# prsinha1/Distributed-Inverse-Problem-Admm

Hardware: AMD Instinct MI355X
Metric: ADMM node-updates/sec (whole node), 512² phantom; rel-Fro vs CPU ref (higher is better)
Workload: dtype f32 samples / f64 state; 1 GPU; C3 (BASELINE.json configs[2] 512^2, 16 graph nodes (ring), 96 angles/node, float32 samples, iso TV, lam=0.02 rho=2, split-Bregman 10x5 CG) on 1 GPU(s), one step = one outer ADMM iteration; image=512, nodes=16, angles_per_node=96, graph=ring, parallelism=graph-node shards x1, batch_streams=1

## Files before the change

distributed-inverse-problem-admm_amd/csrc/admm_tomo.hip:

```cpp
#include <hip/hip_runtime.h>

#include <algorithm>
#include <cmath>
#include <cstdio>
#include <cstdlib>
#include <cstring>
#include <initializer_list>
#include <memory>
#include <string>
#include <type_traits>
#include <utility>
#include <vector>

#include "../../include/admm_tomo.h"
#include "fwd_plan.hpp"
#include "kernels.hpp"

using namespace admm;

static_assert(sizeof(FgBlock) == sizeof(int4) && alignof(FgBlock) == alignof(int4), "FgBlock must be an int4");

namespace {
thread_local std::string g_err;

// ... 145 lines not shown
  int kbias = 0;
  int wexp = 0;
  static constexpr int kPlans = kFwdPlans;
  FwdPlan plans[kPlans];
  Buf plan_groups_b[kPlans], plan_rng_b[kPlans];
  const FgGroup* plan_groups(int pl) const { return plan_groups_b[pl].as<const FgGroup>(); }
  const FgRange* plan_rng(int pl) const { return plan_rng_b[pl].as<const FgRange>(); }
  int plan_n[kPlans] = {}, plan_blocks[kPlans] = {};
  double plan_staged[kPlans] = {};
  const FgGroup* groups = nullptr;
  const FgRange* rng = nullptr;
  int n_groups = 0;
  bool mirror_half = false;
  Buf fg_order;
  int fg_nblk = 0, fg_order_nch = 0;
  int fg_cpb = 1;
  Stream cap;

  bool csr = false;
  long long nnz = 0;
  Buf f_ptr, f_idx, f_val, t_ptr, t_idx, t_val;

  Buf op_img, op_imgT, op_sino, op_fpart;
  Buf op_order[kPlans];
  int op_nblk[kPlans] = {};
  int op_fpart_key = -1;

  bool bound = false;
  admm_batch b{};
  int vb = 1;
  bool mm = false;
  int bk_staging = 0;
  bool bk_epi_lds = true;
  int n_cu = 0;
  std::unique_ptr<admm_ctx> half;
  Buf xs, xsT, p, pT, Hp, sino, bI, fpart, r, c, d2, e2;
  Buf dsumS;
  Buf wS;
  bool weighted = false;
  Buf x2, p2;
  Buf pring;
  Buf ats;
  std::vector<Event>* tf_ev = nullptr;
  size_t tf_next = 0;
  int tf_kind = 0;
  bool ats_valid = false;
  Buf partH, partS, partD, partE;
  Buf redH;
  int P_back = 0, P_tile = 0, P_fwd = 0, P_edge = 0;
  Graph upd, upd_reuse, cons;

  admm_ctx() = default;
  admm_ctx(const admm_ctx&) = delete;
  admm_ctx& operator=(const admm_ctx&) = delete;
  ~admm_ctx() {
    scope.enter(device);
    (void)hipDeviceSynchronize();
    half.reset();
  }
};

namespace {

int vb_for(int V, int dtype) {
  const int vb = V >= 5 ? 8 : (V >= 3 ? 4 : (V == 2 ? 2 : 1));
  return dtype == ADMM_DTYPE_F64 ? std::min(vb, 4) : vb;
// ... 230 lines not shown
    const size_t mthreads = (size_t)mh * (MODE == 0 ? 2 : 1);
    dim3 mg((unsigned)((mthreads + kBlock - 1) / kBlock), nch * (VB / MH));
    with_weights(wts, [&](auto... w) {
      hipLaunchKernelGGL((k_fwd_combine_mirror<T, VBV, VB, MODE, decltype(w)...>), mg, dim3(kBlock), 0, s,
                         (const T*)C->fpart.p, sino, b, part, C->half->fang(), C->g.n_det, C->half->g.n_angles, V, w...);
    });
    CHECK_LAUNCH();
    return ADMM_OK;
  }
  dim3 cg((C->mrays + kBlock - 1) / kBlock, nch);
  with_weights(wts, [&](auto... w) {
    hipLaunchKernelGGL((k_fwd_combine<T, VB, MODE, decltype(w)...>), cg, dim3(kBlock), 0, s, (const T*)C->fpart.p, sino, b,
                       part, C->fang(), C->g.n_det, C->g.n_angles, V, w...);
  });
  CHECK_LAUNCH();
  return ADMM_OK;
}

template <typename T>
void back_geom(BackArgs<T>& a, const admm_ctx* C, const admm_ctx* A, int V) {
  a.ang = A->bang();
  a.angc = A->bangc();
  a.K = A->Kb;
  a.kbias = A->kbias;
  a.wexp = A->wexp;
  a.N = C->g.N;
  a.n_det = C->g.n_det;
  a.n_ang = A->g.n_angles;
  a.V = V;
}

template <typename T, int VB, int MODE>
int launch_back(admm_ctx* C, BackArgs<T> a, int V, hipStream_t s) {
  if constexpr (MODE == BACK_H || MODE == BACK_INIT || MODE == BACK_DIAG || MODE == BACK_ATB) {
    if (C->mm) {
      constexpr int VBV = mirror_vb<T, VB>(), MH = VBV / 2;
      back_geom(a, C, C->half.get(), V);
      const int N = C->g.N, Nh = (N + 1) / 2;
      dim3 grid((N + kBTJ - 1) / kBTJ, (Nh + kBTI - 1) / kBTI, ((V + VB - 1) / VB) * (VB / MH));
      void (*kern)(BackArgs<T>) = k_back_mirror<T, VBV, VB, MODE>;
      if constexpr (back_mirror_dma<T, VBV, MODE>()) {
        if (C->bk_staging == 1) {
          kern = k_back_mirror_reg<T, VBV, VB, MODE>;
        } else if constexpr (std::is_same<T, float>::value) {
          const bool fills = (long)grid.x * grid.y * grid.z >= 2L * C->n_cu;
          if (grid.z % 2 == 0 && (C->bk_staging == 3 || (C->bk_staging == 0 && fills))) {
            kern = C->bk_epi_lds ? k_back_mirror_2<T, VBV, VB> : k_back_mirror_2_gepi<T, VBV, VB>;
            grid.z /= 2;
          } else if (!C->bk_epi_lds) {
            kern = k_back_mirror_gepi<T, VBV, VB, MODE>;
          }
        }
      }
      hipLaunchKernelGGL(kern, grid, dim3(kBkThreads), 0, s, a);
      CHECK_LAUNCH();
      return ADMM_OK;
    }
  }
  back_geom(a, C, C, V);
  const int N = C->g.N;
  constexpr bool kOneImage = MODE == BACK_WSQ || MODE == BACK_WSQW;
  dim3 grid((N + kBTJ - 1) / kBTJ, (N + kBTI - 1) / kBTI, kOneImage ? 1 : (V + VB - 1) / VB);
  if (C->csr) {
    a.csr_ptr = (const int*)C->t_ptr.p;
    a.csr_idx = (const int*)C->t_idx.p;
    a.csr_val = (const T*)C->t_val.p;
    hipLaunchKernelGGL((k_back<T, VB, MODE, true>), grid, dim3(kBkThreads), 0, s, a);
// ... 156 lines not shown
      std::swap(dcur, dnxt);
      std::swap(ecur, enxt);
    }
    std::swap(xcur, xnxt);
    if (!last) std::swap(slot[0], slot[F == 2 ? K : 1]);
  }
  if (xcur != B.x_ext)
    HIPCHK(hipMemcpyAsync(B.x_ext, xcur, (size_t)V * npix * sizeof(double), hipMemcpyDeviceToDevice, s));
  if (dcur != B.d) {
    HIPCHK(hipMemcpyAsync(B.d, dcur, 2 * V * npix * sizeof(double), hipMemcpyDeviceToDevice, s));
    HIPCHK(hipMemcpyAsync(B.e, ecur, 2 * V * npix * sizeof(double), hipMemcpyDeviceToDevice, s));
  }
  RET((launch_fwd_batch<T, VB, 1>(C, xs, xsT, sino, (const T*)B.b, (double*)C->partS.p, V, s)));
  {
    BackArgs<T> a{};
    a.sino = sino;
    a.part = (double*)C->partD.p;
    a.dsum = B.dsum;
    a.cvec = c;
    a.x = B.x_ext;
    a.phantom = B.phantom;
    a.edges = edge_in(B);
    a.qv = B.q;
    a.inc_off = B.inc_off;
    a.inc_edge = B.inc_edge;
    a.inc_qslot = B.inc_qslot;
    a.inc_sign = B.inc_sign;
    a.rho = B.rho;
    a.lam = B.lam;
    a.mu = B.mu;
    a.tv_kind = B.tv_kind;
    a.evar = B.e;
    a.out_t = (B.flags & ADMM_BATCH_KEEP_X) ? (T*)C->ats.p : nullptr;
    RET((launch_back<T, VB, BACK_DIAG>(C, a, V, s)));
  }
  RET(launch_reduce((double*)C->partS.p, V, C->P_fwd, B.node_stats, 1, ADMM_NODE_STATS, ADMM_NODE_STAT_MSE_SINO, s));
  RET(launch_reduce((double*)C->partD.p, 5 * V, Pb, B.node_stats, 5, ADMM_NODE_STATS, ADMM_NODE_STAT_G2, s));
  return ADMM_OK;
}

int enqueue_update_any(admm_ctx* C, hipStream_t s, bool reuse = false, int rounds = 0) {
  return with_type_vb(C->dtype, C->vb, [&](auto tt, auto vbc) {
    return enqueue_update<typename decltype(tt)::type, decltype(vbc)::value>(C, s, reuse, rounds);
  });
}

int cons_rows(int n_xext) { return n_xext <= 16 ? 16 : n_xext <= 64 ? 64 : n_xext <= 128 ? 128 : 0; }

int enqueue_consensus_stored(admm_ctx* C, int e0, int e1, hipStream_t s) {
  const admm_batch& B = C->b;
  if (e1 <= e0) return ADMM_OK;
  const int npix = C->npix;
  dim3 grid((npix + kBlock * 4 - 1) / (kBlock * 4), e1 - e0);
  hipLaunchKernelGGL(k_consensus<false>, grid, dim3(kBlock), 0, s, B.x_ext, B.y, nullptr, B.z, nullptr, B.edge_a,
                     B.edge_b, (double*)C->partE.p, npix, e0);
  CHECK_LAUNCH();
  RET(launch_reduce((double*)C->partE.p + (size_t)3 * e0 * C->P_edge, 3 * (e1 - e0), C->P_edge,
                    B.edge_stats + (size_t)3 * e0, 1, 1, 0, s));
  return ADMM_OK;
}

int enqueue_consensus(admm_ctx* C, hipStream_t s) {
  const admm_batch& B = C->b;
  if (B.n_edges == 0) return ADMM_OK;
  const int npix = C->npix;
  if (B.z == nullptr) {
    const dim3 g((npix + kConsPix - 1) / kConsPix);
// ... 106 lines not shown
  RET(ensure(C->op_sino, vbmax * m * ds));
  RET(ensure(C->op_fpart, (size_t)kFgSeg * vbmax * m * ds));
  for (int v0 = 0; v0 < nimg; v0 += step) {
    const int nc = std::min(step, nimg - v0);
    const T* in = img + (size_t)v0 * npix;
    T* out = sino + (size_t)v0 * m;
    RET(with_vb(vb_for(nc, C->dtype), [&](auto vbc) { return op_forward_chunk<T, decltype(vbc)::value>(C, in, out, nc, s); }));
  }
  return ADMM_OK;
}

}

extern "C" {

int admm_abi_version(void) { return ADMM_ABI_VERSION; }
const char* admm_last_error(void) { return g_err.c_str(); }

int admm_ctx_create(admm_ctx** out, const admm_geom* geom, int dtype, int max_images, int device) {
  if (!out || !geom) return fail(ADMM_E_INVALID, "null argument");
  *out = nullptr;
  const admm_geom g = *geom;
  if (const char* err = check_geom(g, dtype, max_images)) return fail(ADMM_E_INVALID, err);
  GeomTables T;
  if (const char* err = geom_tables(g, dtype, T)) return fail(ADMM_E_INVALID, err);
  FwdPlans P = build_fwd_plans(g, T.fa);
  DEVICE_SCOPE(device);
  std::unique_ptr<admm_ctx> C(new admm_ctx());
  C->g = g;
  C->dtype = dtype;
  C->device = device;
  C->bk_staging = env_word("ADMM_BK_STAGING", {"reg", "dma1", "dma2"});
  C->bk_epi_lds = env_word("ADMM_BK_EPI", {"global"}) == 0;
  HIPCHK(hipDeviceGetAttribute(&C->n_cu, hipDeviceAttributeMultiprocessorCount, device));
  C->max_images = max_images;
  C->npix = g.N * g.N;
  C->mrays = g.n_angles * g.n_det;
  C->Kb = T.Kb;
  C->kbias = T.kbias;
  C->wexp = T.wexp;
  RET(upload(C->fang_b, T.fa));
  RET(upload(C->bang_b, T.ba));
  RET(upload(C->bangc_b, T.bc));
  if (P.fits) {
    for (int pl = 0; pl < admm_ctx::kPlans; ++pl) {
      FwdPlan& Q = P.plan[pl];
      if (Q.groups.empty()) continue;
      RET(upload(C->plan_groups_b[pl], Q.groups));
      RET(upload(C->plan_rng_b[pl], Q.ranges));
      C->plan_n[pl] = (int)Q.groups.size();
      C->plan_blocks[pl] = (int)Q.blocks.size();
      C->plan_staged[pl] = Q.staged;
      C->plans[pl] = std::move(Q);
    }
    select_fwd_plan(C.get(), 0);
  }
  HIPCHK(hipStreamCreateWithFlags(&C->cap.s, hipStreamNonBlocking));
  *out = C.release();
  return ADMM_OK;
}

int admm_ctx_create_matrix(admm_ctx** out, int N, int m, long long nnz, const long long* indptr,
                           const int* indices, const double* values, int dtype, int max_images, int device) {
  if (!out || !indptr || (nnz > 0 && (!indices || !values))) return fail(ADMM_E_INVALID, "null argument");
  *out = nullptr;
  if (N < 2 || N > 4096 || m < 1) return fail(ADMM_E_INVALID, "bad matrix sizes");
// ... 5 lines not shown
    return fail(ADMM_E_INVALID, "batch too large for 32-bit buffer offsets; split it across contexts");
  if (indptr[0] != 0 || indptr[m] != nnz) return fail(ADMM_E_INVALID, "indptr must run from 0 to nnz");
  for (int r = 0; r < m; ++r)
    if (indptr[r + 1] < indptr[r]) return fail(ADMM_E_INVALID, "indptr not non-decreasing");
  for (long long k = 0; k < nnz; ++k)
    if (indices[k] < 0 || (size_t)indices[k] >= npix) return fail(ADMM_E_INVALID, "column index out of range");
  std::vector<int> tptr(npix + 1, 0), tidx((size_t)nnz);
  std::vector<double> tval((size_t)nnz);
  for (long long k = 0; k < nnz; ++k) ++tptr[(size_t)indices[k] + 1];
  for (size_t c = 0; c < npix; ++c) tptr[c + 1] += tptr[c];
  {
    std::vector<int> fill(tptr.begin(), tptr.end() - 1);
    for (int r = 0; r < m; ++r)
      for (long long k = indptr[r]; k < indptr[r + 1]; ++k) {
        const int q = fill[indices[k]]++;
        tidx[q] = r;
        tval[q] = values[k];
      }
  }
  std::vector<int> fptr(m + 1);
  for (int r = 0; r <= m; ++r) fptr[r] = (int)indptr[r];
  DEVICE_SCOPE(device);
  std::unique_ptr<admm_ctx> C(new admm_ctx());
  C->g = admm_geom{};
  C->g.N = N;
  C->g.n_angles = 1;
  C->g.n_det = m;
  C->dtype = dtype;
  C->device = device;
  C->max_images = max_images;
  C->npix = (int)npix;
  C->mrays = m;
  C->csr = true;
  C->nnz = nnz;
  FwdAngle fa{};
  fa.L = 1.0;
  BackAngle ba{};
  BackAngleC bc{};
  auto upv = [&](Buf& b, const std::vector<double>& v) {
    if (dtype == ADMM_DTYPE_F64) return upload(b, v, 16);
    return upload(b, std::vector<float>(v.begin(), v.end()), 16);
  };
  RET(upload(C->f_ptr, fptr, 16));
  RET(upload(C->f_idx, indices, (size_t)nnz * 4, 16));
  RET(upv(C->f_val, std::vector<double>(values, values + nnz)));
  RET(upload(C->t_ptr, tptr, 16));
  RET(upload(C->t_idx, tidx, 16));
  RET(upv(C->t_val, tval));
  RET(upload(C->fang_b, &fa, sizeof(fa)));
  RET(upload(C->bang_b, &ba, sizeof(ba)));
  RET(upload(C->bangc_b, &bc, sizeof(bc)));
  HIPCHK(hipStreamCreateWithFlags(&C->cap.s, hipStreamNonBlocking));
  *out = C.release();
  return ADMM_OK;
}

int admm_ctx_destroy(admm_ctx* C) {
  if (!C) return ADMM_OK;
  delete C;
  return ADMM_OK;
}

int admm_project_fwd(admm_ctx* C, const void* img, void* sino, int nimg, void* stream) {
  if (!C || !img || !sino) return fail(ADMM_E_INVALID, "null argument");
  if (nimg < 1 || nimg > C->max_images) return fail(ADMM_E_INVALID, "nimg out of range");
  hipStream_t s = (hipStream_t)stream;
// ... 384 lines not shown
```

distributed-inverse-problem-admm_amd/csrc/kernels.hpp:

```cpp
#pragma once
#include <hip/hip_runtime.h>
#include <stdint.h>

#include <type_traits>

#include "tables.hpp"

namespace admm {

constexpr int kBlock = 256;
constexpr int kTile = 32;
constexpr int kFwdRays = 64;
constexpr int kFwdSegs = 8;
constexpr int kFwdBlock = kFwdRays * kFwdSegs;


__device__ __forceinline__ int clampi(int v, int lo, int hi) { return min(max(v, lo), hi); }

constexpr double kKfBias = 1048576.0;
constexpr unsigned kKfHi = 0x41300000u;
__device__ __forceinline__ void kf_split(double kfb, unsigned& hi, float& fu) {
  const uint64_t b = __builtin_bit_cast(uint64_t, kfb);
  hi = (unsigned)(b >> 32);
  fu = (float)(unsigned)b;
// ... 1002 lines not shown
        } else {
          lo[u] = T(0);
          hi[u] = T(0);
        }
      } else if constexpr (WT) {
        lo[u] *= wl[u];
        hi[u] *= wh[u];
      }
    }
    T* base = sino + (size_t)rc * m_full * VBR + mq * MH;
    gstore<T, MH>(base + ray * VBR, lo);
    gstore<T, MH>(base + ray2 * VBR, hi);
  }
  if (MODE == 1) {
    __shared__ double lds[4 * MH];
    block_reduce<MH>(sq, lds);
    if (threadIdx.x == 0) {
#pragma unroll
      for (int u = 0; u < MH; ++u)
        if (vr0 + u < V) pout[(size_t)(vr0 + u) * gridDim.x + blockIdx.x] = sq[u];
    }
  }
}

struct EdgeIn {
  const double* z;
  const double* y;
  const double* yb;
  const double* xp;
  const int* ea;
  const int* eb;
};

enum BackMode { BACK_PLAIN = 0, BACK_ATB = 1, BACK_WSQ = 2, BACK_H = 3, BACK_INIT = 4, BACK_DIAG = 5, BACK_WSQW = 6 };

template <typename T>
struct BackArgs {
  const T* sino;
  const BackAngle* ang;
  const BackAngleC* angc;
  double K;
  int kbias;
  int wexp;
  int N, n_det, n_ang, V;
  const int* csr_ptr;
  const int* csr_idx;
  const T* csr_val;
  T* out_t;
  double* out_d;
  double* part;
  const T* pin;
  const double* r;
  const double* dsum;
  const T* dsum_s;
  const double* atb;
  const double* cvec;
  const double* dvar;
  const double* evar;
  const double* x;
  const double* phantom;
  EdgeIn edges;
  const double* qv;
  const int* inc_off;
  const int* inc_edge;
  const int* inc_qslot;
  const int* inc_sign;
  double rho, lam, mu;
// ... 201 lines not shown
    gstore<T, VB>(A.out_t + sbase + (size_t)pix * VS, outv);
  }
}

#ifndef ADMM_BK_TI
#define ADMM_BK_TI 32
#endif
#ifndef ADMM_BK_TJ
#define ADMM_BK_TJ 32
#endif
constexpr int kBTJ = ADMM_BK_TJ;
constexpr int kBTI = ADMM_BK_TI;
constexpr int kBkThreads = kBTJ * kBTI;
constexpr int kBkWaves = kBkThreads / 64;
constexpr int kBkPatchJ = kBTJ / 16;
static_assert((kBTJ == 32 || kBTJ == 64) && kBTI % 4 == 0 && kBkThreads <= 1024 && kBkWaves >= 4,
              "unsupported back-projector tile");
constexpr int ce_isqrt_ceil(int v) {
  int r = 0;
  while (r * r < v) ++r;
  return r;
}
constexpr int kBWin = ((ce_isqrt_ceil((kBTJ - 1) * (kBTJ - 1) + (kBTI - 1) * (kBTI - 1)) + 3 + 7) / 8) * 8;
#ifndef ADMM_BK_ANGC
#define ADMM_BK_ANGC 32
#endif
constexpr int kBAngC = ADMM_BK_ANGC;

#ifndef ADMM_DIAG_G
#define ADMM_DIAG_G 2
#endif
constexpr int kDiagG = ADMM_DIAG_G;
constexpr int kDiagScratch = kDiagG * ((kBTI + 2) * (kBTJ + 2) + 2 * (kBTI + 1) * (kBTJ + 1));
template <typename T, int VB, int VS = VB>
__device__ __forceinline__ void diag_epilogue_tile(const BackArgs<T>& A, double* scratch, int ib, int jb, int i,
                                                   int j, bool inb, int chunk, int v0, int nv, const T (&acc)[VB],
                                                   double (&pq)[VB][5], int lo = 0) {
  constexpr int XC = kBTJ + 2, XR = kBTI + 2, SC = kBTJ + 1, SR = kBTI + 1;
  constexpr int G = kDiagG, XS = XR * XC, SS = SR * SC;
  const int N = A.N, npix = N * N;
  const int pix = i * N + j;
  const size_t sbase = (size_t)chunk * npix * VS + lo;
  if (inb && A.out_t) gstore<T, VB>(A.out_t + sbase + (size_t)pix * VS, acc);
  const int ti = i - ib + 1, tj = j - jb + 1;
#pragma unroll
  for (int u0 = 0; u0 < VB; u0 += G) {
    if (u0 >= nv) break;
    const int ng = min(G, nv - u0);
    __syncthreads();
    for (int q = threadIdx.x; q < ng * XS; q += kBkThreads) {
      const int g = q / XS, e = q % XS;
      const int rr = e / XC, cc = e % XC;
      const int ii = ib - 1 + rr, jj = jb - 1 + cc;
      const double* xv = A.x + (size_t)(v0 + u0 + g) * npix;
      scratch[q] = (ii >= 0 && jj >= 0 && ii < N && jj < N) ? xv[ii * N + jj] : 0.0;
    }
    __syncthreads();
    for (int q = threadIdx.x; q < ng * SS; q += kBkThreads) {
      const int g = q / SS, e = q % SS;
      const int rr = e / SC, cc = e % SC;
      const int ii = ib - 1 + rr, jj = jb - 1 + cc;
      const double* xt = scratch + g * XS;
      double px = 0.0, py = 0.0;
      if (ii >= 0 && jj >= 0 && ii < N && jj < N) {
        const double c = xt[rr * XC + cc];
        const double gx = (ii < N - 1) ? xt[(rr + 1) * XC + cc] - c : 0.0;
        const double gy = (jj < N - 1) ? xt[rr * XC + cc + 1] - c : 0.0;
        tv_sub(gx, gy, A.tv_kind, px, py);
      }
      scratch[G * XS + 2 * g * SS + e] = px;
      scratch[G * XS + (2 * g + 1) * SS + e] = py;
    }
    __syncthreads();
    if (!inb) continue;
#pragma unroll
    for (int g = 0; g < G; ++g) {
      const int u = u0 + g;
      if (u >= VB || g >= ng) break;
      const int v = v0 + u;
      const size_t vo = (size_t)v * npix;
      const double* xt = scratch + g * XS;
      const double* sx = scratch + G * XS + 2 * g * SS;
      const double* sy = sx + SS;
      const double xc = xt[ti * XC + tj];
      const double gx = (i < N - 1) ? xt[(ti + 1) * XC + tj] - xc : 0.0;
      const double gy = (j < N - 1) ? xt[ti * XC + tj + 1] - xc : 0.0;
      const double tvv = (A.tv_kind == 0) ? sqrt(gx * gx + gy * gy) : fabs(gx) + fabs(gy);
      double kts = 0.0;
      if (i <= N - 2) kts -= sx[ti * SC + tj];
      if (j <= N - 2) kts -= sy[ti * SC + tj];
      if (i >= 1) kts += sx[(ti - 1) * SC + tj];
      if (j >= 1) kts += sy[ti * SC + tj - 1];
      const double cc = A.cvec[vo + pix];
      const double sm = (double)acc[u] + A.rho * (A.dsum[vo + pix] * xc - cc);
      const double gg = sm + A.lam * kts;
      const double* ev = A.evar + 2 * vo;
      double kte = 0.0;
      if (i >= 1) kte += ev[pix - N];
      if (i <= N - 2) kte -= ev[pix];
      if (j >= 1) kte += ev[npix + pix - 1];
      if (j <= N - 2) kte -= ev[npix + pix];
      const double rsb = sm + A.mu * kte;
      double quad = 0.0;
      for (int q = A.inc_off[v]; q < A.inc_off[v + 1]; ++q) {
        const double vij = edge_v(A.edges, A.inc_edge[q], A.inc_sign[q], npix, pix);
        const double dd = xc - vij;
        quad += A.qv[(size_t)A.inc_qslot[q] * npix + pix] * dd * dd;
      }
      pq[u][0] += gg * gg;
      pq[u][1] += tvv;
      pq[u][2] += 0.5 * A.rho * quad;
      if (A.phantom) {
        const double dp = xc - A.phantom[pix];
        pq[u][3] += dp * dp;
      }
      pq[u][4] += rsb * rsb;
    }
  }
}

#ifndef ADMM_BK_NARROW_WPE
#define ADMM_BK_NARROW_WPE 1
#endif
template <typename T, int VB, int MODE>
constexpr int back_waves_per_eu() {
  return (std::is_same<T, float>::value && VB <= 4 && (MODE == BACK_H || MODE == BACK_INIT)) ? ADMM_BK_NARROW_WPE : 1;
}
template <typename T, int VB, int MODE, bool CSR = false>
__global__ __launch_bounds__(kBkThreads) __attribute__((amdgpu_waves_per_eu(back_waves_per_eu<T, VB, MODE>())))
void k_back(BackArgs<T> A) {
  constexpr int NQ = (MODE == BACK_H) ? 5 : (MODE == BACK_DIAG) ? 5 : 1;
  constexpr int NPL = Planes<T, VB>::NPL, PV = Planes<T, VB>::PV;
  const int N = A.N, n_det = A.n_det, n_ang = A.n_ang;
  const int m_rays = n_ang * n_det;
  const int jb = blockIdx.x * kBTJ, ib = blockIdx.y * kBTI;
  const int lane = threadIdx.x & 63, wv = threadIdx.x >> 6;
  const int j = jb + 16 * (wv % kBkPatchJ) + (lane & 15);
  const int i = ib + 4 * (wv / kBkPatchJ) + (lane >> 4);
  const bool inb = (i < N) && (j < N);
  const int chunk = blockIdx.z;
  const int v0 = chunk * VB;
  const int nv = (MODE == BACK_WSQ) ? 1 : min(VB, A.V - v0);
  const double c0 = 0.5 * (N - 1);
  const double xi = (double)min(i, N - 1) - c0, yj = (double)min(j, N - 1) - c0;
  const int jhi = min(jb + kBTJ - 1, N - 1), ihi = min(ib + kBTI - 1, N - 1);
  const int kbias = A.kbias;
  const double Kc = A.K + (double)kbias;
  const double Kcb = Kc + kKfBias;
  constexpr bool FB = std::is_same<T, float>::value;

  constexpr int ANGC_ = (NPL > 2) ? kBAngC / 2 : kBAngC;
  constexpr int ANGC_DIAG = (98304 / (NPL * kBWin * (int)sizeof(Pack<T, PV>))) & ~3;
  constexpr int ANGC = (MODE == BACK_DIAG && ANGC_ > ANGC_DIAG) ? ANGC_DIAG : ANGC_;
  static_assert(ANGC % 4 == 0, "angle chunks are read as int4 groups");
  __shared__ Pack<T, PV> win[NPL][(MODE == BACK_WSQ) ? 1 : ANGC][kBWin];
  __shared__ int4 kmin_s[2][ANGC / 4 + 1];
  T acc[VB];
#pragma unroll
  for (int u = 0; u < VB; ++u) acc[u] = T(0);
  const T* sino_c = A.sino + (size_t)chunk * m_rays * VB;
  int t0c = 0;

  constexpr int PB = (int)sizeof(Pack<T, PV>);
  auto tap = [&](const BackAngleC& g, int koff, T& w0, T& w1, Pack<T, PV> (&s0)[NPL], Pack<T, PV> (&s1)[NPL],
                 int tt) {
    int k0, off;
    if constexpr (std::is_same<T, float>::value) {
      k0 = (int)(tap_f32<PB>(fma(xi, g.Bi, fma(yj, g.Bj, Kcb)), g, koff, w0, w1, off) - kKfHi);
    } else {
      k0 = tap_f64(fma(xi, g.Bi, fma(yj, g.Bj, Kc)), A.ang[t0c + tt], w0, w1);
      off = k0 * PB + koff;
    }
    if constexpr (MODE == BACK_WSQ) {
      (void)off;
      w0 = (k0 >= kbias && k0 <= kbias + n_det - 1) ? w0 : T(0);
      w1 = (k0 >= kbias - 1 && k0 <= kbias + n_det - 2) ? w1 : T(0);
    } else {
#pragma unroll
      for (int q = 0; q < NPL; ++q) {
        const char* wb = reinterpret_cast<const char*>(&win[q][0][0]) + off;
        s0[q] = *reinterpret_cast<const Pack<T, PV>*>(wb);
        s1[q] = *reinterpret_cast<const Pack<T, PV>*>(wb + PB);
      }
    }
  };
  auto fmac = [&](T w0, T w1, const Pack<T, PV> (&s0)[NPL], const Pack<T, PV> (&s1)[NPL]) {
// ... 120 lines not shown
      }
    }
    for (; tt < nt; ++tt) {
      const BackAngleC g = A.angc[t0 + tt];
      int km = 0;
      if constexpr (MODE != BACK_WSQ) km = reinterpret_cast<const int*>(kmin_s[kb])[tt];
      T wa0, wa1;
      Pack<T, PV> sa0[NPL], sa1[NPL];
      tap(g, km, wa0, wa1, sa0, sa1, tt);
      fmac(wa0, wa1, sa0, sa1);
    }
    if constexpr (PF) {
      if (t0 + ANGC < n_ang) {
        __syncthreads();
        wcommit(t0 + ANGC);
        kmin_store(t0 + 2 * ANGC, kb, rec2);
        __syncthreads();
      }
    }
  }

  if constexpr (std::is_same<T, float>::value && !CSR) {
    if (A.wexp != 0) {
      const int e = (MODE == BACK_WSQ || MODE == BACK_WSQW) ? 2 * A.wexp : A.wexp;
#pragma unroll
      for (int u = 0; u < VB; ++u) acc[u] = ldexpf(acc[u], e);
    }
  }
  double pq[VB][NQ];
#pragma unroll
  for (int u = 0; u < VB; ++u)
#pragma unroll
    for (int q = 0; q < NQ; ++q) pq[u][q] = 0.0;
  if constexpr (MODE == BACK_DIAG) {
    __shared__ double diag_s[kDiagScratch];
    diag_epilogue_tile<T, VB>(A, diag_s, ib, jb, i, j, inb, chunk, v0, nv, acc, pq);
  } else if (inb) {
    back_epilogue<T, VB, MODE, NQ>(A, i, j, chunk, v0, nv, acc, pq);
  }

  if constexpr (MODE == BACK_H || MODE == BACK_DIAG) {
    constexpr int NT = VB * NQ, NS = RsShape<NT>::NS;
    __shared__ double lds[kBkWaves * NS];
    __shared__ double tot[NS];
    double flat[NT];
#pragma unroll
    for (int u = 0; u < VB; ++u)
#pragma unroll
      for (int q = 0; q < NQ; ++q) flat[u * NQ + q] = pq[u][q];
    block_reduce_flat<NT, kBkWaves>(flat, lds, tot);
    const int t = threadIdx.x;
    if (t < VB * NQ && t / NQ < nv) {
      const int P = gridDim.x * gridDim.y;
      const int b = blockIdx.y * gridDim.x + blockIdx.x;
      A.part[((size_t)v0 * NQ + t) * P + b] = tot[t];
    }
  }
}

template <typename T, int VB, int MODE>
constexpr bool back_mirror_dma() {
  return MODE == BACK_H && Planes<T, VB>::NPL == 2 && sizeof(Pack<T, Planes<T, VB>::PV>) == 16;
}
constexpr int kPtR = kBTI + 2, kPtC = kBTJ + 2, kPtSlots = kPtR * kPtC;
using lds_char = __attribute__((address_space(3))) char;
template <int LB>
constexpr int ptile_bytes() {
  return ((2 * LB * kPtSlots + 63) / 64) * 64 * 16;
}
template <typename T, int VBR, int MH, int LB>
__device__ __forceinline__ void ptile_stage(const BackArgs<T>& A, lds_char* lds, int ib, int jb, int z0) {
  static_assert(MH * sizeof(T) == 16, "one 16-byte slot per pixel and lane block");
  constexpr int MS = VBR / MH, NSLOT = 2 * LB * kPtSlots, NPC = (NSLOT + 63) / 64;
  const int N = A.N, npix = N * N;
  const int lane = threadIdx.x & 63;
  const int wvu = __builtin_amdgcn_readfirstlane((int)threadIdx.x >> 6);
  const uint64_t b = (uint64_t)(uintptr_t)A.pin;
  const uint32_t lo = __builtin_amdgcn_readfirstlane((uint32_t)b);
  const uint32_t hi = __builtin_amdgcn_readfirstlane((uint32_t)(b >> 32));
  const __amdgpu_buffer_rsrc_t rs =
      make_rsrc((const void*)(uintptr_t)(((uint64_t)hi << 32) | lo),
                (uint32_t)((size_t)((A.V + VBR - 1) / VBR) * npix * VBR * sizeof(T)));
  for (int pc = wvu; pc < NPC; pc += kBkWaves) {
    const int q = pc * 64 + lane;
    const int t = q / kPtSlots, s = q - t * kPtSlots, rr = s / kPtC, cc = s - rr * kPtC;
    const int z = z0 + (t >> 1);
    const int row = ((t & 1) ? N - 1 - ib - kBTI : ib - 1) + rr, col = jb - 1 + cc;
    const bool in = q < NSLOT && row >= 0 && row < N && col >= 0 && col < N;
    const unsigned voff =
        in ? (unsigned)(((z / MS) * npix + row * N + col) * VBR + (z % MS) * MH) * (unsigned)sizeof(T) : 0xFFFFFFFFu;
    __builtin_amdgcn_raw_ptr_buffer_load_lds(rs, (__attribute__((address_space(3))) void*)(lds + pc * (64 * 16)), 16,
                                             voff, 0, 0, 0);
  }
}

template <typename T, int VB, int VBR, int MODE, bool DMAQ, bool EPIQ = true, int LB = 1>
__device__ __forceinline__ void back_mirror_body(const BackArgs<T>& A) {
  static_assert(MODE == BACK_H || MODE == BACK_INIT || MODE == BACK_DIAG || MODE == BACK_ATB, "batch modes");
  static_assert(LB == 1 || LB == 2, "one or two lane blocks per block");
  constexpr int MH = VB / 2, MS = VBR / MH;
  static_assert(VB % 2 == 0 && VBR % MH == 0, "mirror: VB = 2 x (a divisor of VBR)");
  constexpr int NQ = (MODE == BACK_H || MODE == BACK_DIAG) ? 5 : 1;
  constexpr int NPL = Planes<T, VB>::NPL, PV = Planes<T, VB>::PV;
  constexpr int PB = (int)sizeof(Pack<T, PV>);
  const int N = A.N, n_det = A.n_det, n_ang = A.n_ang;
  const int Nh = (N + 1) / 2;
  const size_t m_full = (size_t)2 * n_ang * n_det;
  const int jb = blockIdx.x * kBTJ, ib = blockIdx.y * kBTI;
  const int lane = threadIdx.x & 63, wv = threadIdx.x >> 6;
  const int j = jb + 16 * (wv % kBkPatchJ) + (lane & 15);
  const int i = ib + 4 * (wv / kBkPatchJ) + (lane >> 4);
  const int i2 = N - 1 - i;
  const bool inb = (i < Nh) && (j < N);
  const bool inb2 = inb && (i2 != i);
  const int z0 = (int)blockIdx.z * LB;
  const double c0 = 0.5 * (N - 1);
  const double xi = (double)min(i, Nh - 1) - c0, yj = (double)min(j, N - 1) - c0;
  const int jhi = min(jb + kBTJ - 1, N - 1), ihi = min(ib + kBTI - 1, Nh - 1);
  const int kbias = A.kbias;
  const double Kc = A.K + (double)kbias;
  const double Kcb = Kc + kKfBias;
  constexpr bool FB = std::is_same<T, float>::value;
  constexpr int ANGC_ = ((NPL > 2) ? kBAngC / 2 : kBAngC) / (2 * LB);
  constexpr int ANGC_DIAG = (98304 / (2 * NPL * kBWin * PB)) & ~3;
  constexpr int ANGC = (MODE == BACK_DIAG && ANGC_ > ANGC_DIAG) ? ANGC_DIAG : ANGC_;
  static_assert(ANGC % 4 == 0 && ANGC >= 4, "angle chunks are read as int4 groups");
  constexpr bool DMA = DMAQ && back_mirror_dma<T, VB, MODE>();
  static_assert(LB == 1 || (DMA && std::is_same<T, float>::value), "two lane blocks: float32, H mode, LDS-DMA");
  constexpr int NWB = (DMA ? 2 : 1) * LB * 2, NKS = DMA ? 3 : 2;
  constexpr int BUFB = LB * 2 * NPL * ANGC * kBWin * PB;
  constexpr bool EPI = EPIQ && DMA && std::is_same<T, float>::value && MH * sizeof(T) == 16;
  static_assert(!EPI || ptile_bytes<LB>() <= 2 * BUFB, "the p tiles fit in the window array");
  __shared__ Pack<T, PV> win[NWB][NPL][ANGC][kBWin];
  __shared__ int4 kmin_s[NKS][2][ANGC / 4 + 1];
  __shared__ int kst_s[DMA ? 3 : 1][2][DMA ? ANGC + 1 : 1];
  T acc1[LB][VB], acc2[LB][VB];
#pragma unroll
  for (int l = 0; l < LB; ++l)
#pragma unroll
    for (int u = 0; u < VB; ++u) acc1[l][u] = acc2[l][u] = T(0);
  auto sino_lb = [&](int l) { return A.sino + (size_t)((z0 + l) / MS) * m_full * VBR + ((z0 + l) % MS) * MH; };
  int t0c = 0;

  auto kmin_load = [&](int t0) {
    const BackAngleC& g = A.angc[min(t0 + ((int)threadIdx.x % ANGC), n_ang - 1)];
    return make_double2(g.Bi, g.Bj);
  };
  auto kmin_store = [&](int buf, double2 bij, int bo = 0) {
    const int w = (int)threadIdx.x / ANGC;
    const double xa = (double)ib - c0, xb = (double)ihi - c0;
    const double x0 = w ? -xb : xa, x1 = w ? -xa : xb;
    auto kf = [&](double xx, int jj) { return fma(xx, bij.x, fma((double)jj - c0, bij.y, Kc)); };
    const double kmn = fmin(fmin(kf(x0, jb), kf(x0, jhi)), fmin(kf(x1, jb), kf(x1, jhi)));
    const int a = (int)threadIdx.x % ANGC;
    const int k0w = (int)floor(kmn) - 1;
    int koff = (a * kBWin - k0w) * PB;
    if constexpr (FB) koff = (int)((unsigned)koff - kKfHi * (unsigned)PB);
    if constexpr (DMA) {
// ... 165 lines not shown
  const int P = gridDim.x * gridDim.y;
  const int b = blockIdx.y * gridDim.x + blockIdx.x;
  [[maybe_unused]] lds_char* const tb = (lds_char*)&win[0][0][0][0];
  if constexpr (EPI) {
    __syncthreads();
    ptile_stage<T, VBR, MH, LB>(A, tb, ib, jb, z0);
    asm volatile("s_waitcnt vmcnt(0)" ::: "memory");
    __syncthreads();
  }
#pragma unroll
  for (int l = 0; l < LB; ++l) {
    if constexpr (std::is_same<T, float>::value) {
      if (A.wexp != 0) {
#pragma unroll
        for (int u = 0; u < VB; ++u) {
          acc1[l][u] = ldexpf(acc1[l][u], A.wexp);
          acc2[l][u] = ldexpf(acc2[l][u], A.wexp);
        }
      }
    }
    T r1[MH], r2[MH];
#pragma unroll
    for (int h = 0; h < MH; ++h) {
      r1[h] = acc1[l][h] + acc2[l][MH + h];
      r2[h] = acc2[l][h] + acc1[l][MH + h];
    }
    double pq[MH][NQ];
#pragma unroll
    for (int u = 0; u < MH; ++u)
#pragma unroll
      for (int q = 0; q < NQ; ++q) pq[u][q] = 0.0;
    const int z = z0 + l, rc = z / MS, mq = z % MS;
    const int v0 = rc * VBR + mq * MH, nv = min(MH, A.V - v0);
    if constexpr (MODE == BACK_DIAG) {
      __shared__ double diag_s[kDiagScratch];
      diag_epilogue_tile<T, MH, VBR>(A, diag_s, ib, jb, i, j, inb, rc, v0, nv, r1, pq, mq * MH);
      diag_epilogue_tile<T, MH, VBR>(A, diag_s, N - ib - kBTI, jb, i2, j, inb2, rc, v0, nv, r2, pq, mq * MH);
    } else if constexpr (EPI) {
      using PT = PTile<T, MH, kPtC>;
      if (inb)
        back_epilogue<T, MH, MODE, NQ, VBR, false, PT>(A, i, j, rc, v0, nv, r1, pq, mq * MH,
                                                       PT{tb + (2 * l) * kPtSlots * 16, ib - 1, jb - 1});
      if (inb2)
        back_epilogue<T, MH, MODE, NQ, VBR, true, PT>(A, i2, j, rc, v0, nv, r2, pq, mq * MH,
                                                      PT{tb + (2 * l + 1) * kPtSlots * 16, N - 1 - ib - kBTI, jb - 1});
    } else {
      if (inb) back_epilogue<T, MH, MODE, NQ, VBR>(A, i, j, rc, v0, nv, r1, pq, mq * MH);
      if (inb2) back_epilogue<T, MH, MODE, NQ, VBR, true>(A, i2, j, rc, v0, nv, r2, pq, mq * MH);
    }
    if constexpr (MODE == BACK_H || MODE == BACK_DIAG) {
      constexpr int NT = MH * NQ, NS = RsShape<NT>::NS;
      __shared__ double lds[kBkWaves * NS];
      __shared__ double tot[NS];
      double flat[NT];
#pragma unroll
      for (int u = 0; u < MH; ++u)
#pragma unroll
        for (int q = 0; q < NQ; ++q) flat[u * NQ + q] = pq[u][q];
      block_reduce_flat<NT, kBkWaves>(flat, lds, tot);
      const int t = threadIdx.x;
      if (t < NT && t / NQ < nv) A.part[((size_t)v0 * NQ + t) * P + b] = tot[t];
    }
  }
}

template <typename T, int VB, int VBR, int MODE>
__global__ __launch_bounds__(kBkThreads) void k_back_mirror(BackArgs<T> A) {
  back_mirror_body<T, VB, VBR, MODE, true>(A);
}
template <typename T, int VB, int VBR, int MODE>
__global__ __launch_bounds__(kBkThreads) void k_back_mirror_reg(BackArgs<T> A) {
  back_mirror_body<T, VB, VBR, MODE, false>(A);
}
template <typename T, int VB, int VBR, int MODE>
__global__ __launch_bounds__(kBkThreads) void k_back_mirror_gepi(BackArgs<T> A) {
  back_mirror_body<T, VB, VBR, MODE, true, false>(A);
}
template <typename T, int VB, int VBR>
__global__ __launch_bounds__(kBkThreads) void k_back_mirror_2(BackArgs<T> A) {
  back_mirror_body<T, VB, VBR, BACK_H,  true,  true,  2>(A);
}
template <typename T, int VB, int VBR>
__global__ __launch_bounds__(kBkThreads) void k_back_mirror_2_gepi(BackArgs<T> A) {
// ... 648 lines not shown
```

Measured before the change: 2338 node-updates/s.

## Stage edge incidences in LDS and hoist diag epilogue loads via buffer loads

In the diagnostic back-projection epilogue, the per-node edge incidence records (pointers, signs, counts) are staged once per block into shared memory. The per-pixel operand loads (cvec, dsum, e-variables, edge z/y/q values) are then issued up front through raw buffer loads with wave-uniform base addresses. The aim is to cut dependent scalar index chasing and expose more memory-level parallelism in the epilogue. The cost is more registers and LDS, an extra block barrier, and a capped unrolled incidence loop, so occupancy may drop. The old path is kept behind an environment switch.

```diff
diff --git a/distributed-inverse-problem-admm_amd/csrc/admm_tomo.hip b/distributed-inverse-problem-admm_amd/csrc/admm_tomo.hip
--- a/distributed-inverse-problem-admm_amd/csrc/admm_tomo.hip
+++ b/distributed-inverse-problem-admm_amd/csrc/admm_tomo.hip
@@ -201,6 +201,7 @@
   bool mm = false;
   int bk_staging = 0;
   bool bk_epi_lds = true;
+  bool bk_diag_legacy = false;
   int n_cu = 0;
   std::unique_ptr<admm_ctx> half;
   Buf xs, xsT, p, pT, Hp, sino, bI, fpart, r, c, d2, e2;
@@ -497,7 +498,7 @@
 
 template <typename T, int VB, int MODE>
 int launch_back(admm_ctx* C, BackArgs<T> a, int V, hipStream_t s) {
-  if constexpr (MODE == BACK_H || MODE == BACK_INIT || MODE == BACK_DIAG || MODE == BACK_ATB) {
+  if constexpr (MODE == BACK_H || MODE == BACK_INIT || back_is_diag(MODE) || MODE == BACK_ATB) {
     if (C->mm) {
       constexpr int VBV = mirror_vb<T, VB>(), MH = VBV / 2;
       back_geom(a, C, C->half.get(), V);
@@ -720,7 +721,10 @@
     a.tv_kind = B.tv_kind;
     a.evar = B.e;
     a.out_t = (B.flags & ADMM_BATCH_KEEP_X) ? (T*)C->ats.p : nullptr;
-    RET((launch_back<T, VB, BACK_DIAG>(C, a, V, s)));
+    if (C->bk_diag_legacy)
+      RET((launch_back<T, VB, BACK_DIAG_LEGACY>(C, a, V, s)));
+    else
+      RET((launch_back<T, VB, BACK_DIAG>(C, a, V, s)));
   }
   RET(launch_reduce((double*)C->partS.p, V, C->P_fwd, B.node_stats, 1, ADMM_NODE_STATS, ADMM_NODE_STAT_MSE_SINO, s));
   RET(launch_reduce((double*)C->partD.p, 5 * V, Pb, B.node_stats, 5, ADMM_NODE_STATS, ADMM_NODE_STAT_G2, s));
@@ -893,6 +897,7 @@
   C->device = device;
   C->bk_staging = env_word("ADMM_BK_STAGING", {"reg", "dma1", "dma2"});
   C->bk_epi_lds = env_word("ADMM_BK_EPI", {"global"}) == 0;
+  C->bk_diag_legacy = env_word("ADMM_BK_DIAG", {"legacy"}) == 1;
   HIPCHK(hipDeviceGetAttribute(&C->n_cu, hipDeviceAttributeMultiprocessorCount, device));
   C->max_images = max_images;
   C->npix = g.N * g.N;
@@ -964,6 +969,7 @@
   C->npix = (int)npix;
   C->mrays = m;
   C->csr = true;
+  C->bk_diag_legacy = env_word("ADMM_BK_DIAG", {"legacy"}) == 1;
   C->nnz = nnz;
   FwdAngle fa{};
   fa.L = 1.0;
diff --git a/distributed-inverse-problem-admm_amd/csrc/kernels.hpp b/distributed-inverse-problem-admm_amd/csrc/kernels.hpp
--- a/distributed-inverse-problem-admm_amd/csrc/kernels.hpp
+++ b/distributed-inverse-problem-admm_amd/csrc/kernels.hpp
@@ -1058,7 +1058,9 @@
   const int* eb;
 };
 
-enum BackMode { BACK_PLAIN = 0, BACK_ATB = 1, BACK_WSQ = 2, BACK_H = 3, BACK_INIT = 4, BACK_DIAG = 5, BACK_WSQW = 6 };
+enum BackMode { BACK_PLAIN = 0, BACK_ATB = 1, BACK_WSQ = 2, BACK_H = 3, BACK_INIT = 4, BACK_DIAG = 5, BACK_WSQW = 6,
+                BACK_DIAG_LEGACY = 7 };
+constexpr bool back_is_diag(int mode) { return mode == BACK_DIAG || mode == BACK_DIAG_LEGACY; }
 
 template <typename T>
 struct BackArgs {
@@ -1326,10 +1328,115 @@
 #endif
 constexpr int kDiagG = ADMM_DIAG_G;
 constexpr int kDiagScratch = kDiagG * ((kBTI + 2) * (kBTJ + 2) + 2 * (kBTI + 1) * (kBTJ + 1));
-template <typename T, int VB, int VS = VB>
+
+#ifndef ADMM_DIAG_INC_CAP
+#define ADMM_DIAG_INC_CAP 4
+#endif
+#ifndef ADMM_DIAG_INC_HOIST
+#define ADMM_DIAG_INC_HOIST 2
+#endif
+constexpr int kDiagIncCap = ADMM_DIAG_INC_CAP;
+constexpr int kDiagIncHoist = ADMM_DIAG_INC_HOIST;
+static_assert(kDiagIncHoist >= 1 && kDiagIncHoist <= kDiagIncCap, "hoisted incidences are staged ones");
+enum DiagForm { DIAG_LEGACY = 0, DIAG_GROUPED = 1, DIAG_HOISTED = 2 };
+template <typename T, int VB>
+constexpr int diag_form(int mode) {
+  return mode == BACK_DIAG_LEGACY ? DIAG_LEGACY
+         : VB <= 4                ? DIAG_HOISTED
+         : sizeof(T) == 4         ? DIAG_GROUPED
+                                  : DIAG_LEGACY;
+}
+template <int VB>
+struct DiagInc {
+  const double* pa[VB][kDiagIncCap];
+  const double* pb[VB][kDiagIncCap];
+  const double* py[VB][kDiagIncCap];
+  const double* pq[VB][kDiagIncCap];
+  int sign[VB][kDiagIncCap];
+  int off[VB], cnt[VB];
+};
+template <typename T, int VB>
+__device__ __forceinline__ void diag_inc_stage(const BackArgs<T>& A, DiagInc<VB>& S, int v0, int nv) {
+  static_assert(VB * kDiagIncCap <= kBkThreads, "one thread per record");
+  const int u = (int)threadIdx.x / kDiagIncCap, h = (int)threadIdx.x % kDiagIncCap;
+  if (u < nv) {
+    const EdgeIn& E = A.edges;
+    const size_t npix = (size_t)A.N * A.N;
+    const int q0 = A.inc_off[v0 + u], q1 = A.inc_off[v0 + u + 1];
+    if (h == 0) {
+      S.off[u] = q0;
+      S.cnt[u] = q1 - q0;
+    }
+    const double* pa = A.cvec + (size_t)(v0 + u) * npix;
+    const double *pb = pa, *py = pa, *pq = pa;
+    int sg = 0;
+    if (q0 + h < q1) {
+      const int e = A.inc_edge[q0 + h];
+      sg = A.inc_sign[q0 + h];
+      const size_t eo = (size_t)e * npix;
+      pa = E.z ? E.z + eo : E.xp + (size_t)E.ea[e] * npix;
+      pb = E.z ? pa : E.xp + (size_t)E.eb[e] * npix;
+      py = (E.yb != nullptr && sg <= 0 ? E.yb : E.y) + eo;
+      pq = A.qv + (size_t)A.inc_qslot[q0 + h] * npix;
+    }
+    S.pa[u][h] = pa;
+    S.pb[u][h] = pb;
+    S.py[u][h] = py;
+    S.pq[u][h] = pq;
+    S.sign[u][h] = sg;
+  }
+  __syncthreads();
+}
+__device__ __forceinline__ double diag_ld(const double* row, uint32_t bytes, unsigned bo) {
+  const uint64_t b = (uint64_t)(uintptr_t)row;
+  const uint32_t lo = __builtin_amdgcn_readfirstlane((uint32_t)b);
+  const uint32_t hi = __builtin_amdgcn_readfirstlane((uint32_t)(b >> 32));
+  const auto v = __builtin_amdgcn_raw_buffer_load_b64(
+      make_rsrc((const void*)(uintptr_t)(((uint64_t)hi << 32) | lo), bytes), (int)bo, 0, 0);
+  double d;
+  __builtin_memcpy(&d, &v, 8);
+  return d;
+}
+struct DiagEdgeOps {
+  double za, zb, yv, qq;
+};
+template <int VB>
+__device__ __forceinline__ void diag_edge_load(const DiagInc<VB>& S, bool derived, int u, int h, uint32_t bytes,
+                                               unsigned bo, DiagEdgeOps& o) {
+  o.za = diag_ld(S.pa[u][h], bytes, bo);
+  o.zb = derived ? diag_ld(S.pb[u][h], bytes, bo) : 0.0;
+  o.yv = diag_ld(S.py[u][h], bytes, bo);
+  o.qq = diag_ld(S.pq[u][h], bytes, bo);
+}
+__device__ __forceinline__ double diag_edge_v(const EdgeIn& E, const DiagEdgeOps& o, int s) {
+  const double z = E.z ? o.za : (o.za + o.zb) * 0.5;
+  if (E.yb == nullptr) return z - (double)s * o.yv;
+  return z - o.yv;
+}
+struct DiagOps {
+  double cv, ds, e0, e1, e2, e3;
+  DiagEdgeOps ed[kDiagIncHoist];
+};
+template <typename T, int VB>
+__device__ __forceinline__ void diag_ops_load(const BackArgs<T>& A, const DiagInc<VB>& S, int u, int v, int npix,
+                                              unsigned bo, unsigned bo_up, unsigned bo_left, DiagOps& o) {
+  const size_t vo = (size_t)v * npix;
+  const double* ev = A.evar + 2 * vo;
+  const uint32_t bytes = (uint32_t)npix * 8u;
+  o.cv = diag_ld(A.cvec + vo, bytes, bo);
+  o.ds = diag_ld(A.dsum + vo, bytes, bo);
+  o.e0 = diag_ld(ev, bytes, bo_up);
+  o.e1 = diag_ld(ev, bytes, bo);
+  o.e2 = diag_ld(ev + npix, bytes, bo_left);
+  o.e3 = diag_ld(ev + npix, bytes, bo);
+#pragma unroll
+  for (int h = 0; h < kDiagIncHoist; ++h) diag_edge_load<VB>(S, A.edges.z == nullptr, u, h, bytes, bo, o.ed[h]);
+}
+
+template <typename T, int VB, int VS, int DF>
 __device__ __forceinline__ void diag_epilogue_tile(const BackArgs<T>& A, double* scratch, int ib, int jb, int i,
                                                    int j, bool inb, int chunk, int v0, int nv, const T (&acc)[VB],
-                                                   double (&pq)[VB][5], int lo = 0) {
+                                                   double (&pq)[VB][5], int lo, const DiagInc<VB>* inc) {
   constexpr int XC = kBTJ + 2, XR = kBTI + 2, SC = kBTJ + 1, SR = kBTI + 1;
   constexpr int G = kDiagG, XS = XR * XC, SS = SR * SC;
   const int N = A.N, npix = N * N;
@@ -1337,10 +1444,16 @@
   const size_t sbase = (size_t)chunk * npix * VS + lo;
   if (inb && A.out_t) gstore<T, VB>(A.out_t + sbase + (size_t)pix * VS, acc);
   const int ti = i - ib + 1, tj = j - jb + 1;
+  [[maybe_unused]] const unsigned bo = (unsigned)pix * 8u;
 #pragma unroll
   for (int u0 = 0; u0 < VB; u0 += G) {
     if (u0 >= nv) break;
     const int ng = min(G, nv - u0);
+    [[maybe_unused]] DiagOps ops[G];
+    [[maybe_unused]] auto load_ops = [&](int g) {
+      const unsigned bo_up = i >= 1 ? bo - 8u * (unsigned)N : bo, bo_left = j >= 1 ? bo - 8u : bo;
+      if (u0 + g < VB && g < ng) diag_ops_load<T, VB>(A, *inc, u0 + g, v0 + u0 + g, npix, bo, bo_up, bo_left, ops[g]);
+    };
     __syncthreads();
     for (int q = threadIdx.x; q < ng * XS; q += kBkThreads) {
       const int g = q / XS, e = q % XS;
@@ -1367,10 +1480,15 @@
     }
     __syncthreads();
     if (!inb) continue;
+    if constexpr (DF == DIAG_HOISTED) {
+#pragma unroll
+      for (int g = 0; g < G; ++g) load_ops(g);
+    }
 #pragma unroll
     for (int g = 0; g < G; ++g) {
       const int u = u0 + g;
       if (u >= VB || g >= ng) break;
+      if constexpr (DF == DIAG_GROUPED) load_ops(g);
       const int v = v0 + u;
       const size_t vo = (size_t)v * npix;
       const double* xt = scratch + g * XS;
@@ -1385,18 +1503,40 @@
       if (j <= N - 2) kts -= sy[ti * SC + tj];
       if (i >= 1) kts += sx[(ti - 1) * SC + tj];
       if (j >= 1) kts += sy[ti * SC + tj - 1];
-      const double cc = A.cvec[vo + pix];
-      const double sm = (double)acc[u] + A.rho * (A.dsum[vo + pix] * xc - cc);
+      const double* ev = A.evar + 2 * vo;
+      constexpr bool OPS = DF != DIAG_LEGACY;
+      const double cc = OPS ? ops[g].cv : A.cvec[vo + pix];
+      const double sm = (double)acc[u] + A.rho * ((OPS ? ops[g].ds : A.dsum[vo + pix]) * xc - cc);
       const double gg = sm + A.lam * kts;
-      const double* ev = A.evar + 2 * vo;
       double kte = 0.0;
-      if (i >= 1) kte += ev[pix - N];
-      if (i <= N - 2) kte -= ev[pix];
-      if (j >= 1) kte += ev[npix + pix - 1];
-      if (j <= N - 2) kte -= ev[npix + pix];
+      if (i >= 1) kte += OPS ? ops[g].e0 : ev[pix - N];
+      if (i <= N - 2) kte -= OPS ? ops[g].e1 : ev[pix];
+      if (j >= 1) kte += OPS ? ops[g].e2 : ev[npix + pix - 1];
+      if (j <= N - 2) kte -= OPS ? ops[g].e3 : ev[npix + pix];
       const double rsb = sm + A.mu * kte;
       double quad = 0.0;
-      for (int q = A.inc_off[v]; q < A.inc_off[v + 1]; ++q) {
+      int q, q1;
+      if constexpr (DF == DIAG_LEGACY) {
+        q = A.inc_off[v], q1 = A.inc_off[v + 1];
+      } else {
+        const int cnt = __builtin_amdgcn_readfirstlane(inc->cnt[u]);
+#pragma unroll
+        for (int h = 0; h < kDiagIncCap; ++h) {
+          if (h >= cnt) break;
+          DiagEdgeOps eo;
+          if (h < kDiagIncHoist)
+            eo = ops[g].ed[h];
+          else
+            diag_edge_load<VB>(*inc, A.edges.z == nullptr, u, h, (uint32_t)npix * 8u, bo, eo);
+          const double vij = diag_edge_v(A.edges, eo, __builtin_amdgcn_readfirstlane(inc->sign[u][h]));
+          const double dd = xc - vij;
+          quad += eo.qq * dd * dd;
+        }
+        q = __builtin_amdgcn_readfirstlane(inc->off[u]);
+        q1 = q + cnt;
+        q += kDiagIncCap;
+      }
+      for (; q < q1; ++q) {
         const double vij = edge_v(A.edges, A.inc_edge[q], A.inc_sign[q], npix, pix);
         const double dd = xc - vij;
         quad += A.qv[(size_t)A.inc_qslot[q] * npix + pix] * dd * dd;
@@ -1405,7 +1545,7 @@
       pq[u][1] += tvv;
       pq[u][2] += 0.5 * A.rho * quad;
       if (A.phantom) {
-        const double dp = xc - A.phantom[pix];
+        const double dp = xc - (DF == DIAG_LEGACY ? A.phantom[pix] : diag_ld(A.phantom, (uint32_t)npix * 8u, bo));
         pq[u][3] += dp * dp;
       }
       pq[u][4] += rsb * rsb;
@@ -1423,7 +1563,7 @@
 template <typename T, int VB, int MODE, bool CSR = false>
 __global__ __launch_bounds__(kBkThreads) __attribute__((amdgpu_waves_per_eu(back_waves_per_eu<T, VB, MODE>())))
 void k_back(BackArgs<T> A) {
-  constexpr int NQ = (MODE == BACK_H) ? 5 : (MODE == BACK_DIAG) ? 5 : 1;
+  constexpr int NQ = (MODE == BACK_H) ? 5 : back_is_diag(MODE) ? 5 : 1;
   constexpr int NPL = Planes<T, VB>::NPL, PV = Planes<T, VB>::PV;
   const int N = A.N, n_det = A.n_det, n_ang = A.n_ang;
   const int m_rays = n_ang * n_det;
@@ -1445,7 +1585,7 @@
 
   constexpr int ANGC_ = (NPL > 2) ? kBAngC / 2 : kBAngC;
   constexpr int ANGC_DIAG = (98304 / (NPL * kBWin * (int)sizeof(Pack<T, PV>))) & ~3;
-  constexpr int ANGC = (MODE == BACK_DIAG && ANGC_ > ANGC_DIAG) ? ANGC_DIAG : ANGC_;
+  constexpr int ANGC = (back_is_diag(MODE) && ANGC_ > ANGC_DIAG) ? ANGC_DIAG : ANGC_;
   static_assert(ANGC % 4 == 0, "angle chunks are read as int4 groups");
   __shared__ Pack<T, PV> win[NPL][(MODE == BACK_WSQ) ? 1 : ANGC][kBWin];
   __shared__ int4 kmin_s[2][ANGC / 4 + 1];
@@ -1632,14 +1772,17 @@
   for (int u = 0; u < VB; ++u)
 #pragma unroll
     for (int q = 0; q < NQ; ++q) pq[u][q] = 0.0;
-  if constexpr (MODE == BACK_DIAG) {
+  if constexpr (back_is_diag(MODE)) {
     __shared__ double diag_s[kDiagScratch];
-    diag_epilogue_tile<T, VB>(A, diag_s, ib, jb, i, j, inb, chunk, v0, nv, acc, pq);
+    constexpr int DF = diag_form<T, VB>(MODE);
+    __shared__ DiagInc<VB> inc_s;
+    if constexpr (DF != DIAG_LEGACY) diag_inc_stage<T, VB>(A, inc_s, v0, nv);
+    diag_epilogue_tile<T, VB, VB, DF>(A, diag_s, ib, jb, i, j, inb, chunk, v0, nv, acc, pq, 0, &inc_s);
   } else if (inb) {
     back_epilogue<T, VB, MODE, NQ>(A, i, j, chunk, v0, nv, acc, pq);
   }
 
-  if constexpr (MODE == BACK_H || MODE == BACK_DIAG) {
+  if constexpr (MODE == BACK_H || back_is_diag(MODE)) {
     constexpr int NT = VB * NQ, NS = RsShape<NT>::NS;
     __shared__ double lds[kBkWaves * NS];
     __shared__ double tot[NS];
@@ -1696,11 +1839,11 @@
 
 template <typename T, int VB, int VBR, int MODE, bool DMAQ, bool EPIQ = true, int LB = 1>
 __device__ __forceinline__ void back_mirror_body(const BackArgs<T>& A) {
-  static_assert(MODE == BACK_H || MODE == BACK_INIT || MODE == BACK_DIAG || MODE == BACK_ATB, "batch modes");
+  static_assert(MODE == BACK_H || MODE == BACK_INIT || back_is_diag(MODE) || MODE == BACK_ATB, "batch modes");
   static_assert(LB == 1 || LB == 2, "one or two lane blocks per block");
   constexpr int MH = VB / 2, MS = VBR / MH;
   static_assert(VB % 2 == 0 && VBR % MH == 0, "mirror: VB = 2 x (a divisor of VBR)");
-  constexpr int NQ = (MODE == BACK_H || MODE == BACK_DIAG) ? 5 : 1;
+  constexpr int NQ = (MODE == BACK_H || back_is_diag(MODE)) ? 5 : 1;
   constexpr int NPL = Planes<T, VB>::NPL, PV = Planes<T, VB>::PV;
   constexpr int PB = (int)sizeof(Pack<T, PV>);
   const int N = A.N, n_det = A.n_det, n_ang = A.n_ang;
@@ -1723,7 +1866,7 @@
   constexpr bool FB = std::is_same<T, float>::value;
   constexpr int ANGC_ = ((NPL > 2) ? kBAngC / 2 : kBAngC) / (2 * LB);
   constexpr int ANGC_DIAG = (98304 / (2 * NPL * kBWin * PB)) & ~3;
-  constexpr int ANGC = (MODE == BACK_DIAG && ANGC_ > ANGC_DIAG) ? ANGC_DIAG : ANGC_;
+  constexpr int ANGC = (back_is_diag(MODE) && ANGC_ > ANGC_DIAG) ? ANGC_DIAG : ANGC_;
   static_assert(ANGC % 4 == 0 && ANGC >= 4, "angle chunks are read as int4 groups");
   constexpr bool DMA = DMAQ && back_mirror_dma<T, VB, MODE>();
   static_assert(LB == 1 || (DMA && std::is_same<T, float>::value), "two lane blocks: float32, H mode, LDS-DMA");
@@ -1955,10 +2098,14 @@
       for (int q = 0; q < NQ; ++q) pq[u][q] = 0.0;
     const int z = z0 + l, rc = z / MS, mq = z % MS;
     const int v0 = rc * VBR + mq * MH, nv = min(MH, A.V - v0);
-    if constexpr (MODE == BACK_DIAG) {
+    if constexpr (back_is_diag(MODE)) {
       __shared__ double diag_s[kDiagScratch];
-      diag_epilogue_tile<T, MH, VBR>(A, diag_s, ib, jb, i, j, inb, rc, v0, nv, r1, pq, mq * MH);
-      diag_epilogue_tile<T, MH, VBR>(A, diag_s, N - ib - kBTI, jb, i2, j, inb2, rc, v0, nv, r2, pq, mq * MH);
+      constexpr int DF = diag_form<T, MH>(MODE);
+      __shared__ DiagInc<MH> inc_s;
+      if constexpr (DF != DIAG_LEGACY) diag_inc_stage<T, MH>(A, inc_s, v0, nv);
+      diag_epilogue_tile<T, MH, VBR, DF>(A, diag_s, ib, jb, i, j, inb, rc, v0, nv, r1, pq, mq * MH, &inc_s);
+      diag_epilogue_tile<T, MH, VBR, DF>(A, diag_s, N - ib - kBTI, jb, i2, j, inb2, rc, v0, nv, r2, pq, mq * MH,
+                                         &inc_s);
     } else if constexpr (EPI) {
       using PT = PTile<T, MH, kPtC>;
       if (inb)
@@ -1971,7 +2118,7 @@
       if (inb) back_epilogue<T, MH, MODE, NQ, VBR>(A, i, j, rc, v0, nv, r1, pq, mq * MH);
       if (inb2) back_epilogue<T, MH, MODE, NQ, VBR, true>(A, i2, j, rc, v0, nv, r2, pq, mq * MH);
     }
-    if constexpr (MODE == BACK_H || MODE == BACK_DIAG) {
+    if constexpr (MODE == BACK_H || back_is_diag(MODE)) {
       constexpr int NT = MH * NQ, NS = RsShape<NT>::NS;
       __shared__ double lds[kBkWaves * NS];
       __shared__ double tot[NS];
```

Measured after the change: 2342 node-updates/s (median of 2 runs). About the same (+0.2%).
